# xiezhy6/PASTA-GAN-plusplus

Measured on AMD Instinct MI355X. Metric: 512-res try-on images/sec (SynthesisNetwork fwd), higher is better.
Workload: dtype f32

## Files before the change

include/pasta_gan_ops.h:

```cpp
#ifndef PASTA_GAN_OPS_H
#define PASTA_GAN_OPS_H

#include <stdint.h>

#ifdef __cplusplus
extern "C" {
#endif

#define PG_ABI_VERSION 20

enum pg_dtype { PG_F32 = 0, PG_F16 = 1, PG_BF16 = 2, PG_F64 = 3 };

enum pg_error {
    PG_OK = 0,
    PG_ERR_INVALID_ARG = -1,
    PG_ERR_UNSUPPORTED = -2,
    PG_ERR_TOO_LARGE = -3
};

enum pg_act {
    PG_ACT_LINEAR = 1, PG_ACT_RELU = 2, PG_ACT_LRELU = 3, PG_ACT_TANH = 4, PG_ACT_SIGMOID = 5,
    PG_ACT_ELU = 6, PG_ACT_SELU = 7, PG_ACT_SOFTPLUS = 8, PG_ACT_SWISH = 9
};

// ... 119 lines not shown

int64_t pg_conv2d_up2x3_packed_size(int Cout, int Cin);
int pg_conv2d_up2x3_pack_weight(const float* packed, void* packed_x3, int Cout, int Cin, void* stream);
int pg_conv2d_up2x3_forward(const float* x, const float* packed, const void* packed_x3, float* y, int N, int Cin, int H, int W, int Cout,
                            const int64_t ystride[4], const float* in_scale, const float* out_scale, float* edge_column, void* stream);

int64_t pg_conv2d_stem7x3_packed_size(int Cout);
int pg_conv2d_stem7x3_pack_weight(const float* w, void* packed, int Cout, float scale, int flip_hw, void* stream);
int pg_conv2d_stem7x3_forward(const float* x, const void* packed, float* y, int N, int H, int W, int Cout, const int64_t ystride[4],
                              const pg_conv2d_fusion* fusion, void* stream);

int64_t pg_conv2d_s2x3_packed_size(int Cout, int Cin);
int pg_conv2d_s2x3_pack_weight(const float* packed, void* packed_x3, int Cout, int Cin, void* stream);
int pg_conv2d_s2x3_forward(const float* x, const void* packed_x3, float* y, int N, int Cin, int H, int W, int Cout, const int64_t ystride[4],
                           const pg_conv2d_fusion* fusion, void* stream);

int pg_conv1x1_small(const float* x, const float* w, const float* styles, const float* bias, const float* skip, float* y,
                     int N, int Cin, int64_t HW, int Cout, float scale, float clamp, void* stream);

int pg_conv1x1_fold_prep(const float* wm, const float* bm, const float* wh, const float* bh, const float* styles, float* w_out, float* b_out,
                         int N, int Cm, int C, int Cout, void* stream);
int pg_conv1x1_fold_heads(const float* x, const float* x2, const float* w, const float* bias, const float* skip, float* y_a, float* y_b,
                          int N, int C1, int C2, int64_t HW, int Cout, int c_a, int n_skip, float clamp, void* stream);

int pg_conv3x3_fold_head(const float* xa, const float* xb, const float* w, const float* bias, const float* skip, float* y,
                         int N, int C, int H, int W, int Cout, float clamp, void* stream);

int pg_conv3x3_cin1(const float* x, const float* w, float* y, int N, int H, int W, int Cout, float scale, int act, void* stream);

int pg_instance_norm_stats(const float* x, float* mean, float* rstd, int NC, int64_t HW, float eps, void* stream);
// ... 269 lines not shown
```

pasta-gan-plusplus_amd/csrc/conv1x1_fold.hip:

```cpp
#include "pg_common.h"

#ifndef PG_FOLD_MIN_WAVES
#define PG_FOLD_MIN_WAVES 1
#endif
#ifndef PG_FOLD_UNROLL
#define PG_FOLD_UNROLL 8
#endif

namespace {
typedef float f32x4s __attribute__((ext_vector_type(4)));

__global__ __launch_bounds__(256) void conv1x1_fold_prep_kernel(const float* __restrict__ wm, const float* __restrict__ bm, const float* __restrict__ wh,
                                                                const float* __restrict__ bh, const float* __restrict__ styles, float* __restrict__ w_out,
                                                                float* __restrict__ b_out, int Cm, int C, int Cout) {
    const int o = blockIdx.x, n = blockIdx.y;
    const float* who = wh + (int64_t)o * Cm;
    const float* sn = styles ? styles + (int64_t)n * Cm : nullptr;
    for (int c = threadIdx.x; c <= C; c += 256) {
        double acc = 0.0;
        if (c < C) {
            for (int k = 0; k < Cm; k++) acc += (double)who[k] * (double)(sn ? sn[k] : 1.f) * (double)wm[(int64_t)k * C + c];
            w_out[((int64_t)n * Cout + o) * C + c] = (float)acc;
        } else {
            if (bm)
                for (int k = 0; k < Cm; k++) acc += (double)who[k] * (double)(sn ? sn[k] : 1.f) * (double)bm[k];
            b_out[(int64_t)n * Cout + o] = (float)(acc + (double)(bh ? bh[o] : 0.f));
        }
    }
}

template <int CP>
__global__ __launch_bounds__(256, PG_FOLD_MIN_WAVES) void conv1x1_fold_heads_kernel(const float* __restrict__ x, const float* __restrict__ x2, const float* __restrict__ w,
                                                                 const float* __restrict__ bias, const float* __restrict__ skip, float* __restrict__ ya,
// ... 42 lines not shown
#pragma unroll
                for (int e = 0; e < 4; e++) r[e] = fminf(fmaxf(r[e], -cl), cl);
                if (o < n_skip) r += ((const f32x4s*)skip)[((int64_t)n * n_skip + o) * HW4 + p];
                if (o < c_a) ((f32x4s*)ya)[((int64_t)n * c_a + o) * HW4 + p] = r;
                else ((f32x4s*)yb)[((int64_t)n * (Cout - c_a) + (o - c_a)) * HW4 + p] = r;
            }
        }
    }
}
}

PG_EXPORT int pg_conv1x1_fold_prep(const float* wm, const float* bm, const float* wh, const float* bh, const float* styles, float* w_out, float* b_out,
                                   int N, int Cm, int C, int Cout, void* stream) {
    if (!wm || !wh || !w_out || !b_out || N <= 0 || Cm <= 0 || C <= 0 || Cout <= 0) return PG_ERR_INVALID_ARG;
    if (N > 65535) return PG_ERR_TOO_LARGE;
    hipLaunchKernelGGL(conv1x1_fold_prep_kernel, dim3((unsigned)Cout, (unsigned)N), dim3(256), 0, (hipStream_t)stream, wm, bm, wh, bh, styles, w_out, b_out, Cm, C, Cout);
    return pg::launch_status();
}

PG_EXPORT int pg_conv1x1_fold_heads(const float* x, const float* x2, const float* w, const float* bias, const float* skip, float* y_a, float* y_b,
                                    int N, int C1, int C2, int64_t HW, int Cout, int c_a, int n_skip, float clamp, void* stream) {
    if (!x || !w || !bias || !y_a || N <= 0 || C1 <= 0 || C2 < 0 || HW <= 0 || Cout <= 0 || c_a <= 0 || c_a > Cout || n_skip < 0 || n_skip > Cout) return PG_ERR_INVALID_ARG;
    if ((C2 > 0 && !x2) || (c_a < Cout && !y_b) || (n_skip > 0 && !skip)) return PG_ERR_INVALID_ARG;
    const int CP = (Cout + 3) / 4 * 4;
    const size_t lds = (size_t)(C1 + C2) * CP * sizeof(float);
    if (Cout > 16 || HW % 4 != 0 || !pg::aligned16(x) || (C2 > 0 && !pg::aligned16(x2)) || !pg::aligned16(y_a) || (c_a < Cout && !pg::aligned16(y_b)) ||
        (n_skip > 0 && !pg::aligned16(skip)) || lds > 64 * 1024)
        return PG_ERR_UNSUPPORTED;
    if (N > 65535) return PG_ERR_TOO_LARGE;
    const int64_t HW4 = HW / 4;
    int64_t bx = (HW4 + 255) / 256;
// ... 10 lines not shown
```

pasta-gan-plusplus_amd/torch_utils/custom_ops.py:

```python

import concurrent.futures
import ctypes
import fcntl
import glob
import hashlib
import os
import re
import shutil
import subprocess
import sys

verbosity = 'brief'

CSRC_DIR = os.path.normpath(os.path.join(os.path.dirname(os.path.abspath(__file__)), '..', 'csrc'))
INCLUDE_DIR = os.path.normpath(os.path.join(CSRC_DIR, '..', '..', 'include'))
DEV_DIR = os.path.join(CSRC_DIR, 'dev')
OFFLOAD_ARCH = 'gfx950'
HIPCC_FLAGS = ['-O3', '-std=c++17', '-fPIC', '-fvisibility=hidden', f'--offload-arch={OFFLOAD_ARCH}']

PLUGIN_SOURCES = {
    'bias_act_plugin': ['bias_act.hip'],
    'upfirdn2d_plugin': ['upfirdn2d.hip'],
    'patch_routing_plugin': ['patch_routing.hip'],
    'augment_plugin': ['augment.hip'],
    'tryon_plugin': ['tryon.hip'],
    'tryon_front_plugin': ['tryon_front.hip'],
    'train_fetch_plugin': ['train_fetch.hip'],
    'snapshot_grid_plugin': ['snapshot_grid.hip'],
    'vgg_loss_plugin': ['vgg_loss.hip'],
    'image_metrics_plugin': ['image_metrics.hip'],
    'conv2d_plugin': ['conv2d.hip', 'conv2d_inst_k3s1.hip', 'conv2d_inst_k1s1.hip', 'conv2d_inst_k2x2.hip', 'conv2d_inst_k2x1.hip',
                      'conv2d_inst_k1x2.hip', 'conv2d_inst_k7s1.hip', 'conv2d_inst_k3s2.hip', 'conv2d_inst_k1s2.hip', 'conv2d_inst_wino.hip', 'conv2d_inst_wino4.hip', 'conv2d_inst_wino4s.hip', 'conv2d_inst_wino4t.hip', 'conv2d_inst_wino4x.hip', 'conv2d_inst_wino4xs.hip', 'conv2d_inst_wino4xt.hip', 'conv2d_inst_wino4b.hip', 'conv2d_inst_wino4bs.hip', 'conv2d_inst_up2.hip', 'conv2d_inst_stem7.hip', 'conv2d_inst_s2x3.hip', 'conv2d_inst_s1x1.hip',
                      'conv2d_wgrad.hip', 'conv2d16.hip', 'conv2d16_inst_k3s1.hip', 'conv2d16_inst_k3s1b.hip', 'conv2d16_inst_k1s1.hip', 'conv2d16_inst_k2x2.hip', 'conv2d16_inst_k2x1.hip',
                      'conv2d16_inst_k1x2.hip', 'conv2d16_inst_k3s2.hip', 'conv2d16_inst_up2f.hip', 'conv1x1_head16.hip', 'spade16.hip', 'conv1x1_fold.hip', 'conv3x3_fold.hip', 'optim.hip'],
}

ABI_VERSION = 20

_cached_plugins = dict()


class NativePlugin:

    def __init__(self, name, path, abi_name=None):
        self.name = name
        self.path = path
        self.lib = ctypes.CDLL(path)
        probe = getattr(self.lib, 'pg_' + (abi_name or name).replace('_plugin', '') + '_abi_version', None)
        if probe is None:
            raise RuntimeError(f'{path} does not export its ABI version; rebuild it from csrc/')
        probe.restype = ctypes.c_int
        if probe() != ABI_VERSION:
# ... 198 lines not shown
```

pasta-gan-plusplus_amd/torch_utils/ops/conv2d_mfma.py:

```python

import contextlib
import ctypes
import os
import weakref

import torch

from .. import custom_ops
from . import _native as nat

ACT_INDEX = {'linear': 1, 'relu': 2, 'lrelu': 3, 'tanh': 4, 'sigmoid': 5, 'elu': 6, 'selu': 7, 'softplus': 8, 'swish': 9}

FUSED_ACTS = ('linear', 'relu', 'lrelu')

SUPPORTED = {(3, 3, 1), (1, 1, 1), (2, 2, 1), (2, 1, 1), (1, 2, 1), (7, 7, 1), (3, 3, 2), (1, 1, 2)}


class Fusion(ctypes.Structure):
    _fields_ = [
        ('in_scale', ctypes.c_void_p), ('in_bias', ctypes.c_void_p), ('in_act', ctypes.c_int), ('in_alpha', ctypes.c_float),
        ('in_gain', ctypes.c_float), ('in_clamp', ctypes.c_float),
        ('out_scale', ctypes.c_void_p), ('noise', ctypes.c_void_p), ('noise_batch_stride', ctypes.c_int64), ('noise_gain', ctypes.c_float),
        ('bias', ctypes.c_void_p), ('act', ctypes.c_int), ('alpha', ctypes.c_float), ('gain', ctypes.c_float), ('clamp', ctypes.c_float),
        ('residual', ctypes.c_void_p),
# ... 108 lines not shown
        lib.pg_conv2d_up2x3_forward.argtypes = [vp, vp, vp, vp, i, i, i, i, i, ctypes.POINTER(ctypes.c_int64), vp, vp, vp, vp]
        lib.pg_conv2d_up2_forward_splitk.restype = i
        lib.pg_conv2d_up2_forward_splitk.argtypes = [vp, vp, vp, i, i, i, i, i, ctypes.POINTER(ctypes.c_int64), vp, vp, vp, i, vp]
        lib.pg_conv2d_stem7x3_packed_size.restype = i64
        lib.pg_conv2d_stem7x3_packed_size.argtypes = [i]
        lib.pg_conv2d_stem7x3_pack_weight.restype = i
        lib.pg_conv2d_stem7x3_pack_weight.argtypes = [vp, vp, i, ctypes.c_float, i, vp]
        lib.pg_conv2d_stem7x3_forward.restype = i
        lib.pg_conv2d_stem7x3_forward.argtypes = [vp, vp, vp, i, i, i, i, ctypes.POINTER(ctypes.c_int64), ctypes.POINTER(Fusion), vp]
        lib.pg_conv2d_s2x3_packed_size.restype = i64
        lib.pg_conv2d_s2x3_packed_size.argtypes = [i, i]
        lib.pg_conv2d_s2x3_pack_weight.restype = i
        lib.pg_conv2d_s2x3_pack_weight.argtypes = [vp, vp, i, i, vp]
        lib.pg_conv2d_s2x3_forward.restype = i
        lib.pg_conv2d_s2x3_forward.argtypes = [vp, vp, vp, i, i, i, i, i, ctypes.POINTER(i64), ctypes.POINTER(Fusion), vp]
        lib.pg_conv3x3_cin1.restype = i
        lib.pg_conv3x3_cin1.argtypes = [vp, vp, vp, i, i, i, i, f, i, vp]
        lib.pg_conv1x1_small.restype = i
        lib.pg_conv1x1_small.argtypes = [vp] * 6 + [i, i, i64, i, f, f, vp]
        lib.pg_conv1x1_fold_prep.restype = i
        lib.pg_conv1x1_fold_prep.argtypes = [vp] * 7 + [i, i, i, i, vp]
        lib.pg_conv1x1_fold_heads.restype = i
        lib.pg_conv1x1_fold_heads.argtypes = [vp] * 7 + [i, i, i, i64, i, i, i, f, vp]
        lib.pg_conv3x3_fold_head.restype = i
        lib.pg_conv3x3_fold_head.argtypes = [vp] * 6 + [i, i, i, i, i, f, vp]
        _plugin = plugin
    return _plugin


WINO_F2, WINO_F4, WINO_F4B, WINO_F4X3 = 1, 2, 3, 4
# ... 104 lines not shown
    return True


def pack_s2x3(packed32, cout, cin):
    hit = _s2x3_of_pack.get(id(packed32))
    if hit is not None and hit[0]() is packed32:
        return hit[1]
    lib = _init().lib
    x3 = torch.empty([lib.pg_conv2d_s2x3_packed_size(cout, cin)], dtype=torch.uint8, device=packed32.device)
    with torch.cuda.device(packed32.device):
        nat.check(lib.pg_conv2d_s2x3_pack_weight(nat.ptr(packed32), nat.ptr(x3), cout, cin, nat.stream_of(packed32)), 'pg_conv2d_s2x3_pack_weight')
    _s2x3_of_pack[id(packed32)] = (weakref.ref(packed32, lambda r, k=id(packed32): _s2x3_of_pack.pop(k, None)), x3)
    return x3


def conv2d_forward(x, packed, cout, kh, kw, stride=1, pad=(0, 0), out_hw=None, y=None, out_step=(1, 1), out_off=(0, 0),
                   in_scale=None, in_bias=None, in_act='linear', in_alpha=0.0, in_gain=1.0, in_clamp=None,
                   out_scale=None, noise=None, noise_gain=1.0, bias=None, act='linear', alpha=0.0, gain=1.0, clamp=None,
                   residual=None, spade=None, x2=None, winograd=False, stats_eps=None, s2x3=None):
    lib = _init().lib
    form, label, has_stats_tail, _ = _wino_form(winograd)
    x = _f32c(x, 'x')
    n, cin, h, w = x.shape
    cin_split = 0
    if x2 is not None:
        x2 = _f32c(x2, 'x2')
        if x2.shape[0] != n or x2.shape[2:] != x.shape[2:] or cin % 16 != 0:
            raise nat.NativeOpError('conv2d_mfma: x2 must match x in N, H, W and x must have a multiple of 16 channels')
        cin_split, cin = cin, cin + x2.shape[1]
    pad_y, pad_x = pad
    if out_hw is None:
        out_hw = ((h + 2 * pad_y - kh) // stride + 1, (w + 2 * pad_x - kw) // stride + 1)
    oh, ow = out_hw
    ychan = cout // 2 if spade is not None else cout
# ... 50 lines not shown
    stats_part = None
    if stats_eps is not None:
        if not has_stats_tail or spade is not None or in_scale is not None or noise is not None or residual is not None or x2 is not None or in_act != 'linear':
            raise nat.NativeNotCovered('conv2d_mfma: output statistics are gathered by the F(4x4) kernel\'s plain tail only')
        stats_T = lib.pg_conv2d_winograd4_stats_tiles(int(oh), int(ow))
        stats_part = torch.empty([n * cout * stats_T * 2], dtype=torch.float32, device=x.device)
        fz.stats_partial = stats_part.data_ptr()
    with torch.cuda.device(x.device):
        if _timeline is not None:
            ev0, ev1 = torch.cuda.Event(enable_timing=True), torch.cuda.Event(enable_timing=True)
            ev0.record()
        s2x3 = (s2x3 is not False and not form and (kh, kw, int(stride)) == (3, 3, 2) and (int(pad_y), int(pad_x)) == (0, 0) and tuple(out_step) == (1, 1) and tuple(out_off) == (0, 0)
                and (int(oh), int(ow)) == ((h - 3) // 2 + 1, (w - 3) // 2 + 1) and not torch.is_grad_enabled() and residual is None and spade is None and x2 is None
                and in_scale is None and in_bias is None and out_scale is None and noise is None and in_act == 'linear' and float(in_gain) == 1.0 and in_clamp is None
                and act in FUSED_ACTS and s2x3_wanted(n, cin, cout, h, w))
        st = -2
        if s2x3:
            st = lib.pg_conv2d_s2x3_forward(nat.ptr(x), nat.ptr(pack_s2x3(packed, cout, cin)), nat.ptr(y), n, cin, h, w, cout, nat.i64arr(y.stride()), ctypes.byref(fz), nat.stream_of(x))
            s2x3 = st != -2
        if s2x3:
            pass
        elif form:
            if (kh, kw, int(stride)) != (3, 3, 1) or tuple(out_step) != (1, 1) or tuple(out_off) != (0, 0):
                raise nat.NativeOpError('conv2d_mfma: winograd=True needs a 3x3 stride-1 dense-output launch')
            st = lib.pg_conv2d_winograd_forward(form, nat.ptr(x), nat.ptr(packed), nat.ptr(y), n, cin, h, w, cout, int(pad_y), int(pad_x),
                                                int(oh), int(ow), nat.i64arr(y.stride()), ctypes.byref(fz), nat.stream_of(x))
        else:
            ksplit = 1
            if spade is None and x2 is None and os.environ.get('PG_CONV_SPLITK', '1') != '0':
                ksplit = lib.pg_conv2d_splitk_plan(n, cin, int(oh), int(ow), cout, kh, kw, int(stride))
            if ksplit > 1:
                ws = torch.empty([ksplit * n * cout * int(oh) * int(ow)], dtype=torch.float32, device=x.device)
                st = lib.pg_conv2d_forward_splitk(nat.ptr(x), nat.ptr(packed), nat.ptr(y), n, cin, h, w, cout, kh, kw, int(stride), int(pad_y), int(pad_x),
                                                  int(oh), int(ow), nat.i64arr(y.stride()), int(out_step[0]), int(out_step[1]), int(out_off[0]), int(out_off[1]),
                                                  ctypes.byref(fz), nat.ptr(ws), ksplit, nat.stream_of(x))
            else:
                st = lib.pg_conv2d_forward(nat.ptr(x), nat.ptr(packed), nat.ptr(y), n, cin, h, w, cout, kh, kw, int(stride), int(pad_y), int(pad_x),
                                           int(oh), int(ow), nat.i64arr(y.stride()), int(out_step[0]), int(out_step[1]), int(out_off[0]), int(out_off[1]),
                                           ctypes.byref(fz), nat.stream_of(x))
        if _timeline is not None:
            ev1.record()
            _timeline.append(((kh, kw, int(stride), label, f'N{n} {cin}->{cout} {h}x{w}' + (' spade' if spade is not None else '') + (' xf' if in_act != 'linear' else '') + (' mod' if in_scale is not None else '') + (' res' if residual is not None else '') + (' s2x3' if s2x3 else '')), 2.0 * n * cout * oh * ow * cin * kh * kw, ev0, ev1,
                              4 * (x.numel() + (x2.numel() if x2 is not None else 0) + n * ychan * oh * ow)))
    nat.check(st, 'pg_conv2d_forward')
    if stats_part is not None:
        mean = torch.empty([n * cout], dtype=torch.float32, device=x.device)
        rstd = torch.empty_like(mean)
        with torch.cuda.device(x.device):
            st = lib.pg_instance_norm_finish(nat.ptr(stats_part), nat.ptr(mean), nat.ptr(rstd), n * cout, stats_T, int(oh), int(ow), float(stats_eps), nat.stream_of(x))
        nat.check(st, 'pg_instance_norm_finish')
        return y, (mean, rstd)
    return y


def pack_spade_gamma_beta(w_gamma, w_beta, scale_gamma=1.0, scale_beta=1.0, winograd=False):
    c = int(w_gamma.shape[0])
    grp = 32
# ... 539 lines not shown
```

pasta-gan-plusplus_amd/training/networks.py:

```python

import os
from typing import NamedTuple, Optional
import numpy as np
import torch
import torch.nn as nn

from torch_utils import misc
from torch_utils.ops import _native as nat
from torch_utils.ops import bias_act
from torch_utils.ops import conv2d_gradfix
from torch_utils.ops import conv2d_mfma
from torch_utils.ops import conv2d_mfma16
from torch_utils.ops import conv2d_resample
from torch_utils.ops import fma
from torch_utils.ops import upfirdn2d

SQRT_HALF = float(np.sqrt(0.5))


def _needs_graph(*tensors):
    return torch.is_grad_enabled() and any(t is not None and t.requires_grad for t in tensors)


def _fast_ok(x, *others):
# ... 70 lines not shown


def _modconv_fast(x, weight, styles, noise, up, padding, resample_filter, demodulate, flip_weight, cache, epilogue):
    cout, cin, kh, kw = (int(s) for s in weight.shape)
    n, _, h, w = x.shape
    cache = cache if cache is not None else _PackCache()
    ep = dict(epilogue) if epilogue else {}
    dcoefs = None
    if demodulate:
        w2 = cache.get(('w2',), [weight], lambda: conv2d_mfma.modconv_w2(weight))
        dcoefs = conv2d_mfma.modconv_prep(w2, styles, cout)[0]
    if up == 1:
        if not conv2d_mfma.supported(kh, kw, 1):
            return None
        wg = conv2d_mfma.use_winograd(kh, kw, 1, cout, cin, pad=(padding, padding), hw=x.shape[2:], ep=ep)
        packed = cache.get(('plain', flip_weight, wg), [weight], lambda: conv2d_mfma.pack_weight(weight, flip=not flip_weight, winograd=wg))
        return conv2d_mfma.conv2d_forward(x, packed, cout, kh, kw, stride=1, pad=(padding, padding), in_scale=styles,
                                          out_scale=dcoefs, noise=noise, winograd=wg, **ep)
    fw, fh = upfirdn2d._get_filter_size(resample_filter)
    tpad, fir_pad = _up2_geometry(kh, kw, fw, fh, padding)
    out_hw = ((h - 1) * 2 - 2 * tpad[0] + kh, (w - 1) * 2 - 2 * tpad[1] + kw)

    def build():
        wt = weight.detach().transpose(0, 1)
        if flip_weight:
            wt = wt.flip([2, 3])
        return conv2d_mfma.pack_transposed(wt.contiguous(), 2, tpad, (h, w), out_hw)
    if (kh, kw) == (3, 3) and tuple(tpad) == (0, 0) and os.environ.get('PG_UP2_FUSED', '1') != '0':
        packs = cache.get(('up2_fused', flip_weight), [weight], lambda: conv2d_mfma.pack_up2(weight, flip=flip_weight))
        y = conv2d_mfma.conv_up2_forward(x, packs, cout, in_scale=styles, out_scale=dcoefs)
    else:
        phases = cache.get(('up2', flip_weight, h, w), [weight], build)
        if phases is None:
# ... 1633 lines not shown
```

Before: 296.3.

## Add split-K bf16x3 MFMA kernel for small-resolution 3x3 modulated convs

Adds a dedicated 3x3 stride-1 conv kernel for feature maps of 16x16 or smaller. It uses bf16 three-way split MFMA to keep f32-level accuracy, tiles pixels across batch images, and splits the channel reduction across blocks through a workspace, with a plan function keyed on CU count. Modulated synthesis layers at low resolution are routed to it instead of Winograd or the generic path, aiming to fill the GPU better on small layers. Separately, the fold-prep kernel is split over a third grid dimension with 64-thread blocks for more parallelism. The split-K path adds workspace allocation and reduction overhead, and may add numeric differences.

Measured after the change: 298.5, median of 6. About the same (+0.8%).

```diff
diff --git a/include/pasta_gan_ops.h b/include/pasta_gan_ops.h
--- a/include/pasta_gan_ops.h
+++ b/include/pasta_gan_ops.h
@@ -7,7 +7,7 @@
 extern "C" {
 #endif
 
-#define PG_ABI_VERSION 20
+#define PG_ABI_VERSION 21
 
 enum pg_dtype { PG_F32 = 0, PG_F16 = 1, PG_BF16 = 2, PG_F64 = 3 };
 
@@ -157,6 +157,12 @@
 int pg_conv2d_s2x3_pack_weight(const float* packed, void* packed_x3, int Cout, int Cin, void* stream);
 int pg_conv2d_s2x3_forward(const float* x, const void* packed_x3, float* y, int N, int Cin, int H, int W, int Cout, const int64_t ystride[4],
                            const pg_conv2d_fusion* fusion, void* stream);
+
+int64_t pg_conv2d_small_x3_packed_size(int Cout, int Cin);
+int pg_conv2d_small_x3_pack_weight(const float* packed, void* packed_x3, int Cout, int Cin, void* stream);
+int pg_conv2d_small_x3_plan(int N, int Cin, int H, int W, int Cout, int cus);
+int pg_conv2d_small_x3_forward(const float* x, const void* packed_x3, float* y, int N, int Cin, int H, int W, int Cout, const int64_t ystride[4],
+                               const pg_conv2d_fusion* fusion, float* ws, int shares, void* stream);
 
 int pg_conv1x1_small(const float* x, const float* w, const float* styles, const float* bias, const float* skip, float* y,
                      int N, int Cin, int64_t HW, int Cout, float scale, float clamp, void* stream);
diff --git a/pasta-gan-plusplus_amd/csrc/conv1x1_fold.hip b/pasta-gan-plusplus_amd/csrc/conv1x1_fold.hip
--- a/pasta-gan-plusplus_amd/csrc/conv1x1_fold.hip
+++ b/pasta-gan-plusplus_amd/csrc/conv1x1_fold.hip
@@ -10,13 +10,14 @@
 namespace {
 typedef float f32x4s __attribute__((ext_vector_type(4)));
 
-__global__ __launch_bounds__(256) void conv1x1_fold_prep_kernel(const float* __restrict__ wm, const float* __restrict__ bm, const float* __restrict__ wh,
-                                                                const float* __restrict__ bh, const float* __restrict__ styles, float* __restrict__ w_out,
-                                                                float* __restrict__ b_out, int Cm, int C, int Cout) {
+constexpr int PREP_COLS = 64;
+__global__ __launch_bounds__(PREP_COLS) void conv1x1_fold_prep_kernel(const float* __restrict__ wm, const float* __restrict__ bm, const float* __restrict__ wh,
+                                                                      const float* __restrict__ bh, const float* __restrict__ styles, float* __restrict__ w_out,
+                                                                      float* __restrict__ b_out, int Cm, int C, int Cout) {
     const int o = blockIdx.x, n = blockIdx.y;
     const float* who = wh + (int64_t)o * Cm;
     const float* sn = styles ? styles + (int64_t)n * Cm : nullptr;
-    for (int c = threadIdx.x; c <= C; c += 256) {
+    for (int c = (int)blockIdx.z * PREP_COLS + (int)threadIdx.x; c <= C; c += (int)gridDim.z * PREP_COLS) {
         double acc = 0.0;
         if (c < C) {
             for (int k = 0; k < Cm; k++) acc += (double)who[k] * (double)(sn ? sn[k] : 1.f) * (double)wm[(int64_t)k * C + c];
@@ -89,7 +90,9 @@
                                    int N, int Cm, int C, int Cout, void* stream) {
     if (!wm || !wh || !w_out || !b_out || N <= 0 || Cm <= 0 || C <= 0 || Cout <= 0) return PG_ERR_INVALID_ARG;
     if (N > 65535) return PG_ERR_TOO_LARGE;
-    hipLaunchKernelGGL(conv1x1_fold_prep_kernel, dim3((unsigned)Cout, (unsigned)N), dim3(256), 0, (hipStream_t)stream, wm, bm, wh, bh, styles, w_out, b_out, Cm, C, Cout);
+    int64_t zb = ((int64_t)C + 1 + PREP_COLS - 1) / PREP_COLS;
+    if (zb > 65535) zb = 65535;
+    hipLaunchKernelGGL(conv1x1_fold_prep_kernel, dim3((unsigned)Cout, (unsigned)N, (unsigned)zb), dim3(PREP_COLS), 0, (hipStream_t)stream, wm, bm, wh, bh, styles, w_out, b_out, Cm, C, Cout);
     return pg::launch_status();
 }
 
diff --git a/pasta-gan-plusplus_amd/csrc/conv2d_inst_smallx3.hip b/pasta-gan-plusplus_amd/csrc/conv2d_inst_smallx3.hip
--- /dev/null
+++ b/pasta-gan-plusplus_amd/csrc/conv2d_inst_smallx3.hip
@@ -0,0 +1,43 @@
+#include "conv2d_small_x3.h"
+
+PG_EXPORT int64_t pg_conv2d_small_x3_packed_size(int Cout, int Cin) {
+    if (Cout <= 0 || Cin <= 0 || Cin % 16 != 0) return 0;
+    return pgconv::small_x3_packed_bytes(Cout, Cin);
+}
+
+PG_EXPORT int pg_conv2d_small_x3_pack_weight(const float* packed, void* packed_x3, int Cout, int Cin, void* stream) {
+    if (!packed || !packed_x3 || Cout <= 0 || Cin <= 0 || (((uintptr_t)packed_x3) & 15) != 0) return PG_ERR_INVALID_ARG;
+    if (Cin % 16 != 0) return PG_ERR_UNSUPPORTED;
+    const int CoutP32 = (Cout + 31) / 32 * 32;
+    const int64_t total = (int64_t)((Cin / 16 + 1) & ~1) * 16 * 9 * CoutP32;
+    int64_t blocks = (total + 255) / 256;
+    if (blocks > (int64_t)pg::max_stream_blocks()) blocks = pg::max_stream_blocks();
+    hipLaunchKernelGGL(pgconv::small_x3_pack_kernel, dim3((unsigned)blocks), dim3(256), 0, (hipStream_t)stream, packed, (unsigned short*)packed_x3, Cin, CoutP32);
+    return pg::launch_status();
+}
+
+PG_EXPORT int pg_conv2d_small_x3_plan(int N, int Cin, int H, int W, int Cout, int cus) { return pgconv::small_x3_plan(N, Cin, H, W, Cout, cus); }
+
+PG_EXPORT int pg_conv2d_small_x3_forward(const float* x, const void* packed_x3, float* y, int N, int Cin, int H, int W, int Cout, const int64_t ystride[4],
+                                         const pg_conv2d_fusion* fusion, float* ws, int shares, void* stream) {
+    if (!x || !packed_x3 || !y || !ystride || N <= 0 || Cin <= 0 || H <= 0 || W <= 0 || Cout <= 0) return PG_ERR_INVALID_ARG;
+    if ((((uintptr_t)x) & 3) != 0 || (((uintptr_t)packed_x3) & 15) != 0) return PG_ERR_INVALID_ARG;
+    pgconv::SmallX3Params p;
+    p.x = x; p.y = y; p.ws = ws; p.wx3 = (const unsigned char*)packed_x3;
+    p.in_scale = p.out_scale = p.noise = p.bias = nullptr;
+    p.noise_bs = 0; p.noise_gain = 0.f;
+    p.N = N; p.Cin = Cin; p.H = H; p.W = W; p.Cout = Cout; p.shares = shares;
+    for (int i = 0; i < 4; i++) p.ys[i] = ystride[i];
+    p.act = PG_ACT_LINEAR; p.alpha = 0.f; p.gain = 1.f; p.clamp = -1.f;
+    if (fusion) {
+        const pg_conv2d_fusion& f = *fusion;
+        if (f.in_bias || (f.in_act != 0 && f.in_act != PG_ACT_LINEAR) || f.in_clamp >= 0.f || (f.in_gain != 0.f && f.in_gain != 1.f) || f.residual ||
+            f.spade_x || f.spade_mean || f.spade_rstd || f.x2 || f.stats_partial)
+            return PG_ERR_UNSUPPORTED;
+        const int act = f.act == 0 ? PG_ACT_LINEAR : f.act;
+        if (act != PG_ACT_LINEAR && act != PG_ACT_RELU && act != PG_ACT_LRELU) return PG_ERR_UNSUPPORTED;
+        p.in_scale = f.in_scale; p.out_scale = f.out_scale; p.noise = f.noise; p.noise_bs = f.noise_batch_stride; p.noise_gain = f.noise_gain;
+        p.bias = f.bias; p.act = act; p.alpha = f.alpha; p.gain = f.gain == 0.f ? 1.f : f.gain; p.clamp = f.clamp;
+    }
+    return pgconv::launch_small_x3(p, (hipStream_t)stream);
+}
diff --git a/pasta-gan-plusplus_amd/csrc/conv2d_small_x3.h b/pasta-gan-plusplus_amd/csrc/conv2d_small_x3.h
--- /dev/null
+++ b/pasta-gan-plusplus_amd/csrc/conv2d_small_x3.h
@@ -0,0 +1,362 @@
+#pragma once
+#include <type_traits>
+#include "conv2d_kernel.h"
+
+namespace pgconv {
+
+constexpr int SM_KC = 16;
+constexpr int SM_TM = 32, SM_TN = 128;
+constexpr int SM_MAXHW = 16;
+constexpr int SM_NREC = 164;
+constexpr int SM_ZREC = 162;
+constexpr int SM_PLB = 2 * SM_NREC * 16;
+constexpr int SM_BUF = 3 * SM_PLB;
+constexpr int SM_STAB = 4096;
+constexpr size_t SM_LDS = 4 * (size_t)SM_BUF + SM_STAB * 4;
+constexpr int SM_FRAG = 64 * 16;
+constexpr int SM_WSLAB = 27 * SM_FRAG;
+constexpr int SM_MAX_SHARES = 8;
+
+struct SmallX3Params {
+    const float* x; float* y; float* ws; const unsigned char* wx3;
+    const float *in_scale, *out_scale, *noise, *bias;
+    int64_t noise_bs; float noise_gain;
+    int N, Cin, H, W, Cout, CoutP;
+    int total;
+    int ctiles, mblocks, shares, rounds;
+    int64_t ys[4];
+    int act; float alpha, gain, clamp;
+};
+
+typedef __bf16 sm_bf16x8 __attribute__((ext_vector_type(8)));
+typedef unsigned sm_u32x4 __attribute__((ext_vector_type(4)));
+
+__device__ __forceinline__ void sm_split_pair(float va, float vb, unsigned& p0, unsigned& p1, unsigned& p2) {
+    const unsigned ua = __float_as_uint(va), ub = __float_as_uint(vb);
+    const float ra = va - __uint_as_float(ua & 0xffff0000u), rb = vb - __uint_as_float(ub & 0xffff0000u);
+    const unsigned ura = __float_as_uint(ra), urb = __float_as_uint(rb);
+    const float la = ra - __uint_as_float(ura & 0xffff0000u), lb = rb - __uint_as_float(urb & 0xffff0000u);
+    p0 = __builtin_amdgcn_perm(ub, ua, 0x07060302u);
+    p1 = __builtin_amdgcn_perm(urb, ura, 0x07060302u);
+    p2 = __builtin_amdgcn_perm(__float_as_uint(lb), __float_as_uint(la), 0x07060302u);
+}
+
+__device__ __forceinline__ float sm_tail(const SmallX3Params& p, float v, int n, int co, float nz, float slope, float cl) {
+    const float sc = p.out_scale ? p.out_scale[(int64_t)n * p.Cout + co] : 1.f;
+    const float bi = p.bias ? p.bias[co] : 0.f;
+    v = v * sc + nz + bi;
+    v = v > 0.f ? v : v * slope;
+    return fminf(fmaxf(v * p.gain, -cl), cl);
+}
+
+__global__ __launch_bounds__(256, 1) void conv2d_small_x3(SmallX3Params p) {
+    extern __shared__ __attribute__((aligned(16))) unsigned char sm_smem[];
+    unsigned char* planes = sm_smem;
+    float* stab = (float*)(sm_smem + 4 * SM_BUF);
+
+    const int t = (int)threadIdx.x;
+    const int wave = __builtin_amdgcn_readfirstlane(t >> 6);
+    const int lane = t & 63;
+    const int kg = wave >> 1, cg = wave & 1;
+    const int half = lane >> 5, l31 = lane & 31;
+    const int HW = p.H * p.W;
+    const int nchunks = p.Cin / SM_KC;
+    const int nchp = (nchunks + 1) & ~1;
+
+    const int G = (int)gridDim.x, q8 = G >> 3, r8 = G & 7, xcd = (int)blockIdx.x & 7;
+    int L = (xcd < r8 ? xcd * (q8 + 1) : r8 * (q8 + 1) + (xcd - r8) * q8) + ((int)blockIdx.x >> 3);
+    const int ct = L % p.ctiles; L /= p.ctiles;
+    const int sh = L % p.shares;
+    const int mb = L / p.shares;
+    const int r0 = sh * p.rounds / p.shares, r1 = (sh + 1) * p.rounds / p.shares;
+    const int col0 = ct * SM_TN;
+    const int qlo = col0 - (p.W + 1);
+    const int nrec = SM_TN + 2 * (p.W + 1);
+    const int ch0 = r0 * 2 * SM_KC;
+    const int ch1 = r1 * 2 * SM_KC < p.Cin ? r1 * 2 * SM_KC : p.Cin;
+    const int nch = ch1 - ch0;
+    const int n_lo = (qlo > 0 ? qlo : 0) / HW;
+    const int n_hi = (qlo + nrec - 1 < p.total - 1 ? qlo + nrec - 1 : p.total - 1) / HW;
+
+    for (int i = t; i < (n_hi - n_lo + 1) * nch; i += 256) {
+        const int n = n_lo + i / nch, c = ch0 + i % nch;
+        stab[i] = p.in_scale ? p.in_scale[(int64_t)n * p.Cin + c] : 1.f;
+    }
+    if (t < 24) {
+        const int b = t / 6, rem = t % 6;
+        *(sm_u32x4*)(planes + (size_t)b * SM_BUF + (size_t)(rem >> 1) * SM_PLB + (size_t)((rem & 1) * SM_NREC + SM_ZREC) * 16) = (sm_u32x4){0u, 0u, 0u, 0u};
+    }
+
+    const int tg = cg * 64 + lane;
+    int xoff[3], soff[3], dsto[3];
+    bool tvalid[3], inimg[3];
+#pragma unroll
+    for (int i = 0; i < 3; i++) {
+        const int task = tg + 128 * i;
+        const int kh = task >= nrec ? 1 : 0, rec = task - kh * nrec;
+        tvalid[i] = task < 2 * nrec;
+        const int q = qlo + rec;
+        inimg[i] = tvalid[i] && q >= 0 && q < p.total;
+        const int qq = inimg[i] ? q : 0;
+        const int n = qq / HW, pix = qq - n * HW;
+        xoff[i] = inimg[i] ? (n * p.Cin + kh * 8) * HW + pix : 0;
+        soff[i] = (inimg[i] ? (n - n_lo) * nch + kh * 8 : 0) - ch0;
+        dsto[i] = (kh * SM_NREC + rec) * 16;
+    }
+    float v[3][8];
+    auto prefetch = [&](int c) __attribute__((always_inline)) {
+#pragma unroll
+        for (int i = 0; i < 3; i++)
+#pragma unroll
+            for (int j = 0; j < 8; j++) v[i][j] = p.x[xoff[i] + (c * SM_KC + j) * HW];
+    };
+    auto split_store = [&](int buf, int c) __attribute__((always_inline)) {
+        unsigned char* pb = planes + (size_t)(buf * 2 + kg) * SM_BUF;
+#pragma unroll
+        for (int i = 0; i < 3; i++) {
+            if (tvalid[i]) {
+                const float* sp = stab + soff[i] + c * SM_KC;
+                const f32x4 s0 = *(const f32x4*)sp, s1 = *(const f32x4*)(sp + 4);
+                sm_u32x4 pl[3];
+#pragma unroll
+                for (int j = 0; j < 4; j++) {
+                    const float sa = j < 2 ? s0[2 * j] : s1[2 * j - 4], sb = j < 2 ? s0[2 * j + 1] : s1[2 * j - 3];
+                    const float va = inimg[i] ? v[i][2 * j] * sa : 0.f, vb = inimg[i] ? v[i][2 * j + 1] * sb : 0.f;
+                    unsigned p0, p1, p2;
+                    sm_split_pair(va, vb, p0, p1, p2);
+                    pl[0][j] = p0; pl[1][j] = p1; pl[2][j] = p2;
+                }
+                *(sm_u32x4*)(pb + dsto[i]) = pl[0];
+                *(sm_u32x4*)(pb + SM_PLB + dsto[i]) = pl[1];
+                *(sm_u32x4*)(pb + 2 * SM_PLB + dsto[i]) = pl[2];
+            }
+        }
+    };
+
+    unsigned bbase[2], bmask[2];
+    const unsigned zoff = (unsigned)(half * SM_NREC + SM_ZREC) * 16u;
+#pragma unroll
+    for (int a = 0; a < 2; a++) {
+        const int col = cg * 64 + a * 32 + l31;
+        const int q = col0 + col;
+        const bool ok = q < p.total;
+        const int qq = ok ? q : 0;
+        const int pix = qq % HW, y = pix / p.W, x = pix - y * p.W;
+        unsigned m = 0;
+#pragma unroll
+        for (int tp = 0; tp < 9; tp++) {
+            const int iy = y + tp / 3 - 1, ix = x + tp % 3 - 1;
+            if (ok && iy >= 0 && iy < p.H && ix >= 0 && ix < p.W) m |= 1u << tp;
+        }
+        bmask[a] = m;
+        bbase[a] = (unsigned)(half * SM_NREC + col) * 16u;
+    }
+
+    f32x16 acc[2], accs[2];
+#pragma unroll
+    for (int a = 0; a < 2; a++)
+#pragma unroll
+        for (int k = 0; k < 16; k++) acc[a][k] = accs[a][k] = 0.f;
+    sm_u32x4 A[9][3];
+    auto wslab = [&](int c) __attribute__((always_inline)) {
+        return p.wx3 + ((int64_t)mb * nchp + c) * (int64_t)SM_WSLAB + lane * 16;
+    };
+
+    __syncthreads();
+    auto dchunk = [&](int c) __attribute__((always_inline)) { return c < nchunks ? c : nchunks - 1; };
+    {
+        const int c = 2 * r0 + kg;
+        prefetch(dchunk(c));
+        const unsigned char* w0 = wslab(c);
+#pragma unroll
+        for (int tp = 0; tp < 9; tp++)
+#pragma unroll
+            for (int pl = 0; pl < 3; pl++) A[tp][pl] = *(const sm_u32x4*)(w0 + (tp * 3 + pl) * SM_FRAG);
+        split_store(0, dchunk(c));
+    }
+    auto weights_home = [&]() __attribute__((always_inline)) {
+        __builtin_amdgcn_s_waitcnt(0x0f70);
+#pragma unroll
+        for (int tp = 0; tp < 9; tp++)
+#pragma unroll
+            for (int pl = 0; pl < 3; pl++) asm volatile("" : "+v"(A[tp][pl]));
+    };
+    __syncthreads();
+    weights_home();
+
+    auto round = [&](int r, auto has_next_t) __attribute__((always_inline)) {
+        constexpr bool has_next = decltype(has_next_t)::value;
+        const int buf = (r - r0) & 1;
+        const int c = 2 * r + kg;
+        if (has_next) prefetch(dchunk(c + 2));
+        {
+            const unsigned char* wn = wslab(has_next ? c + 2 : c);
+            const unsigned char* pb = planes + (size_t)(buf * 2 + kg) * SM_BUF;
+            auto b_frag = [&](int tp, int a, int pl) __attribute__((always_inline)) {
+                const unsigned off = ((bmask[a] >> tp) & 1u) ? bbase[a] + (unsigned)((tp / 3) * p.W + tp % 3) * 16u : zoff;
+                return *(const sm_u32x4*)(pb + (size_t)pl * SM_PLB + off);
+            };
+            constexpr int PA[6] = {2, 1, 1, 0, 0, 0}, PB[6] = {0, 1, 0, 2, 1, 0};
+            sm_u32x4 B[2][3];
+            f32x16 accp[2];
+#pragma unroll
+            for (int a = 0; a < 2; a++)
+#pragma unroll
+                for (int k = 0; k < 16; k++) accp[a][k] = 0.f;
+#pragma unroll
+            for (int pl = 0; pl < 3; pl++) B[0][pl] = b_frag(0, 0, pl);
+#pragma unroll
+            for (int tp = 0; tp < 9; tp++) {
+#pragma unroll
+                for (int a = 0; a < 2; a++) {
+                    if (a == 0 || tp + 1 < 9) {
+#pragma unroll
+                        for (int pl = 0; pl < 3; pl++) B[a ^ 1][pl] = a == 0 ? b_frag(tp, 1, pl) : b_frag(tp + 1, 0, pl);
+                    }
+                    __builtin_amdgcn_sched_barrier(0);
+#pragma unroll
+                    for (int pr = 0; pr < 6; pr++) {
+                        f32x16& dacc = pr == 5 ? accp[a] : accs[a];
+                        dacc = __builtin_amdgcn_mfma_f32_32x32x16_bf16(__builtin_bit_cast(sm_bf16x8, A[tp][PA[pr]]), __builtin_bit_cast(sm_bf16x8, B[a][PB[pr]]), dacc, 0, 0, 0);
+                    }
+                    __builtin_amdgcn_sched_barrier(0);
+                }
+                if (has_next) {
+#pragma unroll
+                    for (int pl = 0; pl < 3; pl++) A[tp][pl] = *(const sm_u32x4*)(wn + (tp * 3 + pl) * SM_FRAG);
+                }
+                __builtin_amdgcn_sched_barrier(0);
+            }
+#pragma unroll
+            for (int a = 0; a < 2; a++)
+#pragma unroll
+                for (int k = 0; k < 16; k++) acc[a][k] += accp[a][k];
+        }
+        if (has_next) split_store(buf ^ 1, dchunk(c + 2));
+        __syncthreads();
+        if (has_next) weights_home();
+    };
+    for (int r = r0; r + 1 < r1; r++) round(r, std::true_type());
+    round(r1 - 1, std::false_type());
+
+    float* red = (float*)sm_smem;
+    if (kg == 1) {
+#pragma unroll
+        for (int a = 0; a < 2; a++)
+#pragma unroll
+            for (int k = 0; k < 16; k++) red[((cg * 2 + a) * 16 + k) * 64 + lane] = acc[a][k] + accs[a][k];
+    }
+    __syncthreads();
+    if (kg == 1) return;
+
+    const float cl = p.clamp >= 0.f ? p.clamp : __builtin_inff();
+    const float slope = act_slope(p.act, p.alpha);
+#pragma unroll
+    for (int a = 0; a < 2; a++) {
+        const int q = col0 + cg * 64 + a * 32 + l31;
+        if (q >= p.total) continue;
+        const int n = q / HW, pix = q - n * HW;
+        const int oy = pix / p.W, ox = pix - oy * p.W;
+        if (p.shares > 1) {
+#pragma unroll
+            for (int k = 0; k < 16; k++) {
+                const int co = mb * SM_TM + (k & 3) + 8 * (k >> 2) + 4 * half;
+                const float s = (acc[a][k] + accs[a][k]) + red[((cg * 2 + a) * 16 + k) * 64 + lane];
+                p.ws[((int64_t)sh * p.CoutP + co) * p.total + q] = s;
+            }
+        } else {
+            const float nz = p.noise ? p.noise[n * p.noise_bs + pix] * p.noise_gain : 0.f;
+            float* yp = p.y + (int64_t)n * p.ys[0] + (int64_t)oy * p.ys[2] + (int64_t)ox * p.ys[3];
+#pragma unroll
+            for (int k = 0; k < 16; k++) {
+                const int co = mb * SM_TM + (k & 3) + 8 * (k >> 2) + 4 * half;
+                const float s = (acc[a][k] + accs[a][k]) + red[((cg * 2 + a) * 16 + k) * 64 + lane];
+                if (co < p.Cout) yp[(int64_t)co * p.ys[1]] = sm_tail(p, s, n, co, nz, slope, cl);
+            }
+        }
+    }
+}
+
+__global__ __launch_bounds__(256) void small_x3_finish_kernel(SmallX3Params p) {
+    const int HW = p.H * p.W;
+    const float cl = p.clamp >= 0.f ? p.clamp : __builtin_inff();
+    const float slope = act_slope(p.act, p.alpha);
+    const int64_t total = (int64_t)p.Cout * p.total;
+    for (int64_t i = (int64_t)blockIdx.x * 256 + threadIdx.x; i < total; i += (int64_t)gridDim.x * 256) {
+        const int co = (int)(i / p.total), q = (int)(i - (int64_t)co * p.total);
+        float s = p.ws[(int64_t)co * p.total + q];
+        for (int z = 1; z < p.shares; z++) s += p.ws[((int64_t)z * p.CoutP + co) * p.total + q];
+        const int n = q / HW, pix = q - n * HW;
+        const int oy = pix / p.W, ox = pix - oy * p.W;
+        const float nz = p.noise ? p.noise[n * p.noise_bs + pix] * p.noise_gain : 0.f;
+        p.y[(int64_t)n * p.ys[0] + (int64_t)co * p.ys[1] + (int64_t)oy * p.ys[2] + (int64_t)ox * p.ys[3]] = sm_tail(p, s, n, co, nz, slope, cl);
+    }
+}
+
+__global__ __launch_bounds__(256) void small_x3_pack_kernel(const float* __restrict__ wp32, unsigned short* __restrict__ out, int Cin, int CoutP32) {
+    const int nchp = (Cin / SM_KC + 1) & ~1;
+    const int64_t total = (int64_t)nchp * SM_KC * 9 * CoutP32;
+    for (int64_t i = (int64_t)blockIdx.x * 256 + threadIdx.x; i < total; i += (int64_t)gridDim.x * 256) {
+        const int co = (int)(i % CoutP32), tap = (int)((i / CoutP32) % 9), ci = (int)(i / ((int64_t)CoutP32 * 9));
+        const float v = ci < Cin ? wp32[i] : 0.f;
+        const unsigned u0 = __float_as_uint(v) & 0xffff0000u;
+        const float r = v - __uint_as_float(u0);
+        const unsigned u1 = __float_as_uint(r) & 0xffff0000u;
+        const unsigned u2 = __float_as_uint(r - __uint_as_float(u1)) & 0xffff0000u;
+        const int mb = co >> 5, m = co & 31, chunk = ci >> 4, kh = (ci >> 3) & 1, j = ci & 7;
+        const int64_t dst = (((((int64_t)mb * nchp + chunk) * 9 + tap) * 3) * 2 + kh) * 256 + m * 8 + j;
+        out[dst] = (unsigned short)(u0 >> 16);
+        out[dst + 512] = (unsigned short)(u1 >> 16);
+        out[dst + 1024] = (unsigned short)(u2 >> 16);
+    }
+}
+
+inline int64_t small_x3_packed_bytes(int Cout, int Cin) { return (int64_t)((Cout + SM_TM - 1) / SM_TM) * ((Cin / SM_KC + 1) & ~1) * SM_WSLAB; }
+
+inline int small_x3_plan(int N, int Cin, int H, int W, int Cout, int cus) {
+    if (N <= 0 || Cin <= 0 || H <= 0 || W <= 0 || Cout <= 0 || cus <= 0 || Cin % SM_KC != 0) return 0;
+    const int64_t tiles = (((int64_t)N * H * W + SM_TN - 1) / SM_TN) * ((Cout + SM_TM - 1) / SM_TM);
+    const int rounds = (Cin / SM_KC + 1) / 2;
+    int64_t s = (cus + tiles - 1) / tiles;
+    if (s > rounds / 2) s = rounds / 2;
+    if (s > SM_MAX_SHARES) s = SM_MAX_SHARES;
+    return s < 1 ? 1 : (int)s;
+}
+
+inline bool small_x3_serves(const SmallX3Params& p) {
+    if (p.H < 1 || p.W < 1 || p.H > SM_MAXHW || p.W > SM_MAXHW || p.Cin % SM_KC != 0 || p.Cin < 2 * SM_KC) return false;
+    if ((int64_t)p.N * p.Cin * p.H * p.W >= 0x7fffffffLL / 4 || (int64_t)p.N * p.H * p.W * ((p.Cout + 31) / 32 * 32) >= 0x7fffffffLL / 4) return false;
+    return true;
+}
+
+inline int launch_small_x3(SmallX3Params p, hipStream_t s) {
+    if (!small_x3_serves(p) || !p.wx3) return PG_ERR_UNSUPPORTED;
+    const int nchunks = p.Cin / SM_KC;
+    p.CoutP = (p.Cout + SM_TM - 1) / SM_TM * SM_TM;
+    p.total = p.N * p.H * p.W;
+    p.ctiles = (p.total + SM_TN - 1) / SM_TN;
+    p.mblocks = p.CoutP / SM_TM;
+    p.rounds = (nchunks + 1) / 2;
+    if (p.shares < 1 || p.shares > p.rounds || p.shares > SM_MAX_SHARES) return PG_ERR_INVALID_ARG;
+    if (p.shares > 1 && !p.ws) return PG_ERR_INVALID_ARG;
+    const int HW = p.H * p.W;
+    int ns = (SM_TN + 2 * (p.W + 1) - 1) / HW + 2;
+    if (ns > p.N) ns = p.N;
+    const int share_ch = ((p.rounds + p.shares - 1) / p.shares) * 2 * SM_KC;
+    if ((int64_t)ns * (share_ch < p.Cin ? share_ch : p.Cin) > SM_STAB) return PG_ERR_UNSUPPORTED;
+    const int64_t blocks = (int64_t)p.ctiles * p.mblocks * p.shares;
+    if (blocks > 0x7fffffffLL) return PG_ERR_TOO_LARGE;
+    static PerDeviceOnce once;
+    const hipError_t e = once.run([] { return hipFuncSetAttribute((const void*)conv2d_small_x3, hipFuncAttributeMaxDynamicSharedMemorySize, 160 * 1024); });
+    if (e != hipSuccess) return (int)e;
+    hipLaunchKernelGGL(conv2d_small_x3, dim3((unsigned)blocks), dim3(256), SM_LDS, s, p);
+    int st = launch_status();
+    if (st != 0 || p.shares == 1) return st;
+    const int64_t outs = (int64_t)p.Cout * p.total;
+    int64_t fb = (outs + 255) / 256;
+    if (fb > (int64_t)max_stream_blocks()) fb = max_stream_blocks();
+    hipLaunchKernelGGL(small_x3_finish_kernel, dim3((unsigned)fb), dim3(256), 0, s, p);
+    return launch_status();
+}
+
+}
diff --git a/pasta-gan-plusplus_amd/torch_utils/custom_ops.py b/pasta-gan-plusplus_amd/torch_utils/custom_ops.py
--- a/pasta-gan-plusplus_amd/torch_utils/custom_ops.py
+++ b/pasta-gan-plusplus_amd/torch_utils/custom_ops.py
@@ -30,12 +30,12 @@
     'vgg_loss_plugin': ['vgg_loss.hip'],
     'image_metrics_plugin': ['image_metrics.hip'],
     'conv2d_plugin': ['conv2d.hip', 'conv2d_inst_k3s1.hip', 'conv2d_inst_k1s1.hip', 'conv2d_inst_k2x2.hip', 'conv2d_inst_k2x1.hip',
-                      'conv2d_inst_k1x2.hip', 'conv2d_inst_k7s1.hip', 'conv2d_inst_k3s2.hip', 'conv2d_inst_k1s2.hip', 'conv2d_inst_wino.hip', 'conv2d_inst_wino4.hip', 'conv2d_inst_wino4s.hip', 'conv2d_inst_wino4t.hip', 'conv2d_inst_wino4x.hip', 'conv2d_inst_wino4xs.hip', 'conv2d_inst_wino4xt.hip', 'conv2d_inst_wino4b.hip', 'conv2d_inst_wino4bs.hip', 'conv2d_inst_up2.hip', 'conv2d_inst_stem7.hip', 'conv2d_inst_s2x3.hip', 'conv2d_inst_s1x1.hip',
+                      'conv2d_inst_k1x2.hip', 'conv2d_inst_k7s1.hip', 'conv2d_inst_k3s2.hip', 'conv2d_inst_k1s2.hip', 'conv2d_inst_wino.hip', 'conv2d_inst_wino4.hip', 'conv2d_inst_wino4s.hip', 'conv2d_inst_wino4t.hip', 'conv2d_inst_wino4x.hip', 'conv2d_inst_wino4xs.hip', 'conv2d_inst_wino4xt.hip', 'conv2d_inst_wino4b.hip', 'conv2d_inst_wino4bs.hip', 'conv2d_inst_up2.hip', 'conv2d_inst_stem7.hip', 'conv2d_inst_s2x3.hip', 'conv2d_inst_smallx3.hip', 'conv2d_inst_s1x1.hip',
                       'conv2d_wgrad.hip', 'conv2d16.hip', 'conv2d16_inst_k3s1.hip', 'conv2d16_inst_k3s1b.hip', 'conv2d16_inst_k1s1.hip', 'conv2d16_inst_k2x2.hip', 'conv2d16_inst_k2x1.hip',
                       'conv2d16_inst_k1x2.hip', 'conv2d16_inst_k3s2.hip', 'conv2d16_inst_up2f.hip', 'conv1x1_head16.hip', 'spade16.hip', 'conv1x1_fold.hip', 'conv3x3_fold.hip', 'optim.hip'],
 }
 
-ABI_VERSION = 20
+ABI_VERSION = 21
 
 _cached_plugins = dict()
 
diff --git a/pasta-gan-plusplus_amd/torch_utils/ops/conv2d_mfma.py b/pasta-gan-plusplus_amd/torch_utils/ops/conv2d_mfma.py
--- a/pasta-gan-plusplus_amd/torch_utils/ops/conv2d_mfma.py
+++ b/pasta-gan-plusplus_amd/torch_utils/ops/conv2d_mfma.py
@@ -146,6 +146,14 @@
         lib.pg_conv2d_s2x3_pack_weight.argtypes = [vp, vp, i, i, vp]
         lib.pg_conv2d_s2x3_forward.restype = i
         lib.pg_conv2d_s2x3_forward.argtypes = [vp, vp, vp, i, i, i, i, i, ctypes.POINTER(i64), ctypes.POINTER(Fusion), vp]
+        lib.pg_conv2d_small_x3_packed_size.restype = i64
+        lib.pg_conv2d_small_x3_packed_size.argtypes = [i, i]
+        lib.pg_conv2d_small_x3_pack_weight.restype = i
+        lib.pg_conv2d_small_x3_pack_weight.argtypes = [vp, vp, i, i, vp]
+        lib.pg_conv2d_small_x3_plan.restype = i
+        lib.pg_conv2d_small_x3_plan.argtypes = [i] * 6
+        lib.pg_conv2d_small_x3_forward.restype = i
+        lib.pg_conv2d_small_x3_forward.argtypes = [vp, vp, vp, i, i, i, i, i, ctypes.POINTER(i64), ctypes.POINTER(Fusion), vp, i, vp]
         lib.pg_conv3x3_cin1.restype = i
         lib.pg_conv3x3_cin1.argtypes = [vp, vp, vp, i, i, i, i, f, i, vp]
         lib.pg_conv1x1_small.restype = i
@@ -280,10 +288,52 @@
     return x3
 
 
+_small_x3_of_pack = {}
+_cus_of_device = {}
+
+
+def small_x3_wanted(n, cin, cout, h, w):
+    if os.environ.get('PG_SMALL_X3', '1') == '0' or cin % 16 != 0 or cin < 32 or not (1 <= h <= 16 and 1 <= w <= 16):
+        return False
+    return True
+
+
+def small_x3_layer(n, cin, cout, h, w, pad, ep=None):
+    ep = ep or {}
+    mode = _algo_override[-1] if _algo_override else os.environ.get('PG_CONV_ALGO', 'auto')
+    pad = (pad, pad) if isinstance(pad, int) else tuple(int(v) for v in pad)
+    return (mode == 'auto' and pad == (1, 1) and not torch.is_grad_enabled() and ep.get('residual') is None and ep.get('act', 'linear') in FUSED_ACTS
+            and small_x3_wanted(int(n), int(cin), int(cout), int(h), int(w)))
+
+
+def pack_small_x3(packed32, cout, cin):
+    hit = _small_x3_of_pack.get(id(packed32))
+    if hit is not None and hit[0]() is packed32:
+        return hit[1]
+    lib = _init().lib
+    x3 = torch.empty([lib.pg_conv2d_small_x3_packed_size(cout, cin)], dtype=torch.uint8, device=packed32.device)
+    with torch.cuda.device(packed32.device):
+        nat.check(lib.pg_conv2d_small_x3_pack_weight(nat.ptr(packed32), nat.ptr(x3), cout, cin, nat.stream_of(packed32)), 'pg_conv2d_small_x3_pack_weight')
+    _small_x3_of_pack[id(packed32)] = (weakref.ref(packed32, lambda r, k=id(packed32): _small_x3_of_pack.pop(k, None)), x3)
+    return x3
+
+
+def small_x3_plan(n, cin, cout, h, w, cus):
+    return int(_init().lib.pg_conv2d_small_x3_plan(int(n), int(cin), int(h), int(w), int(cout), int(cus)))
+
+
+def _cus(device):
+    idx = torch.device(device).index
+    idx = torch.cuda.current_device() if idx is None else idx
+    if idx not in _cus_of_device:
+        _cus_of_device[idx] = int(torch.cuda.get_device_properties(idx).multi_processor_count)
+    return _cus_of_device[idx]
+
+
 def conv2d_forward(x, packed, cout, kh, kw, stride=1, pad=(0, 0), out_hw=None, y=None, out_step=(1, 1), out_off=(0, 0),
                    in_scale=None, in_bias=None, in_act='linear', in_alpha=0.0, in_gain=1.0, in_clamp=None,
                    out_scale=None, noise=None, noise_gain=1.0, bias=None, act='linear', alpha=0.0, gain=1.0, clamp=None,
-                   residual=None, spade=None, x2=None, winograd=False, stats_eps=None, s2x3=None):
+                   residual=None, spade=None, x2=None, winograd=False, stats_eps=None, s2x3=None, small_x3=False):
     lib = _init().lib
     form, label, has_stats_tail, _ = _wino_form(winograd)
     x = _f32c(x, 'x')
@@ -364,11 +414,22 @@
                 and (int(oh), int(ow)) == ((h - 3) // 2 + 1, (w - 3) // 2 + 1) and not torch.is_grad_enabled() and residual is None and spade is None and x2 is None
                 and in_scale is None and in_bias is None and out_scale is None and noise is None and in_act == 'linear' and float(in_gain) == 1.0 and in_clamp is None
                 and act in FUSED_ACTS and s2x3_wanted(n, cin, cout, h, w))
+        sx3 = (small_x3 is True and not form and (kh, kw, int(stride)) == (3, 3, 1) and tuple(out_step) == (1, 1) and tuple(out_off) == (0, 0) and (int(oh), int(ow)) == (h, w)
+               and spade is None and x2 is None and in_bias is None and in_act == 'linear' and float(in_gain) == 1.0 and in_clamp is None and stats_eps is None
+               and small_x3_layer(n, cin, cout, h, w, (pad_y, pad_x), dict(residual=residual, act=act)))
         st = -2
-        if s2x3:
+        if sx3:
+            shares = lib.pg_conv2d_small_x3_plan(n, cin, h, w, cout, _cus(x.device))
+            ws = torch.empty([shares * ((cout + 31) // 32 * 32) * n * h * w], dtype=torch.float32, device=x.device) if shares > 1 else None
+            st = lib.pg_conv2d_small_x3_forward(nat.ptr(x), nat.ptr(pack_small_x3(packed, cout, cin)), nat.ptr(y), n, cin, h, w, cout, nat.i64arr(y.stride()), ctypes.byref(fz),
+                                                nat.ptr(ws), shares, nat.stream_of(x)) if shares >= 1 else -2
+            sx3 = st != -2
+        if sx3:
+            pass
+        elif s2x3:
             st = lib.pg_conv2d_s2x3_forward(nat.ptr(x), nat.ptr(pack_s2x3(packed, cout, cin)), nat.ptr(y), n, cin, h, w, cout, nat.i64arr(y.stride()), ctypes.byref(fz), nat.stream_of(x))
             s2x3 = st != -2
-        if s2x3:
+        if sx3 or s2x3:
             pass
         elif form:
             if (kh, kw, int(stride)) != (3, 3, 1) or tuple(out_step) != (1, 1) or tuple(out_off) != (0, 0):
@@ -390,7 +451,7 @@
                                            ctypes.byref(fz), nat.stream_of(x))
         if _timeline is not None:
             ev1.record()
-            _timeline.append(((kh, kw, int(stride), label, f'N{n} {cin}->{cout} {h}x{w}' + (' spade' if spade is not None else '') + (' xf' if in_act != 'linear' else '') + (' mod' if in_scale is not None else '') + (' res' if residual is not None else '') + (' s2x3' if s2x3 else '')), 2.0 * n * cout * oh * ow * cin * kh * kw, ev0, ev1,
+            _timeline.append(((kh, kw, int(stride), label, f'N{n} {cin}->{cout} {h}x{w}' + (' spade' if spade is not None else '') + (' xf' if in_act != 'linear' else '') + (' mod' if in_scale is not None else '') + (' res' if residual is not None else '') + (' s2x3' if s2x3 else '') + (' sx3' if sx3 else '')), 2.0 * n * cout * oh * ow * cin * kh * kw, ev0, ev1,
                               4 * (x.numel() + (x2.numel() if x2 is not None else 0) + n * ychan * oh * ow)))
     nat.check(st, 'pg_conv2d_forward')
     if stats_part is not None:
diff --git a/pasta-gan-plusplus_amd/training/networks.py b/pasta-gan-plusplus_amd/training/networks.py
--- a/pasta-gan-plusplus_amd/training/networks.py
+++ b/pasta-gan-plusplus_amd/training/networks.py
@@ -108,9 +108,12 @@
         if not conv2d_mfma.supported(kh, kw, 1):
             return None
         wg = conv2d_mfma.use_winograd(kh, kw, 1, cout, cin, pad=(padding, padding), hw=x.shape[2:], ep=ep)
+        sx3 = (kh, kw) == (3, 3) and conv2d_mfma.small_x3_layer(n, cin, cout, h, w, padding, ep)
+        if sx3:
+            wg = 0
         packed = cache.get(('plain', flip_weight, wg), [weight], lambda: conv2d_mfma.pack_weight(weight, flip=not flip_weight, winograd=wg))
         return conv2d_mfma.conv2d_forward(x, packed, cout, kh, kw, stride=1, pad=(padding, padding), in_scale=styles,
-                                          out_scale=dcoefs, noise=noise, winograd=wg, **ep)
+                                          out_scale=dcoefs, noise=noise, winograd=wg, small_x3=sx3, **ep)
     fw, fh = upfirdn2d._get_filter_size(resample_filter)
     tpad, fir_pad = _up2_geometry(kh, kw, fw, fh, padding)
     out_hw = ((h - 1) * 2 - 2 * tpad[0] + kh, (w - 1) * 2 - 2 * tpad[1] + kw)
```
